# LeoQLi/DeepSIR

Hardware: AMD Instinct MI355X
Metric: registered pairs/sec (5k-pt 3DMatch-shaped synthetic pairs, 5 registration iterations, KNN pyramid included) (higher is better)
Workload: dtype f32 (GEMMs as fp16-pair MFMA, fp32 accumulate; index decisions exact fp32)

## Files before the change

deepsir_amd/csrc/kernels.h:

```cpp
#pragma once
#include <hip/hip_runtime.h>
#include <stdint.h>
#include <stdlib.h>

namespace dsir {

constexpr int kKnn = 16;

const char* tuning_env(const char* name);
inline bool tuning_flag(const char* name) { return tuning_env(name) != nullptr; }
inline long long tuning_int(const char* name, long long dflt) { const char* e = tuning_env(name); return e ? atoll(e) : dflt; }

#ifndef DSIR_GN_WORDS_DEFINED
#define DSIR_GN_WORDS_DEFINED
constexpr int kGnWords = 4;
#endif
struct GnRef {
  const double* stats;
  const float* gamma;
  const float* beta;
  int groups;
  double inv_count;
};

// ... 176 lines not shown
  Seg in = {};
  const float *W1 = nullptr;
  const float *W2 = nullptr, *b2 = nullptr;
  const float *W3 = nullptr, *b3 = nullptr;
  const float *W4 = nullptr, *b4 = nullptr;
  int ncls = 0, M = 0, clouds = 1;
  float* feat_out = nullptr;
  float* logits_out = nullptr;
  const void* Wh[4] = {nullptr, nullptr, nullptr, nullptr};
  const void* Wl[4] = {nullptr, nullptr, nullptr, nullptr};
};
bool launch_head_mlp(const HeadArgs& a, bool split, hipStream_t st);

struct AggArgs {
  const float* xyz = nullptr; int64_t xyz_cs = 0;
  const float* score = nullptr;
  const float* F = nullptr;
  const float *W1 = nullptr, *b1 = nullptr;
  const float *W2 = nullptr, *b2 = nullptr;
  const float *W3 = nullptr, *b3 = nullptr;
  const float *W4 = nullptr, *b4 = nullptr;
  const float *W5 = nullptr, *b5 = nullptr;
  const float *W6 = nullptr, *b6 = nullptr;
  float* desc = nullptr;
  int n = 0, clouds = 0;
  float* sq = nullptr;
  void* hi = nullptr;
  void* lo = nullptr;
  unsigned long long* packed_init = nullptr;
  const void* Wh[5] = {nullptr, nullptr, nullptr, nullptr, nullptr};
  const void* Wl[5] = {nullptr, nullptr, nullptr, nullptr, nullptr};
};
bool launch_agg_chain(const AggArgs& a, bool split, hipStream_t st);

struct FeatChainArgs {
  const float* X = nullptr;
  const float *W1 = nullptr, *b1 = nullptr;
  const float *W2 = nullptr, *b2 = nullptr;
  const float *W3 = nullptr, *b3 = nullptr;
  const void *W3h = nullptr, *W3l = nullptr;
  float* out0 = nullptr;
  float* out1 = nullptr;
  int split_cloud = 0;
  int n = 0, clouds = 0;
  int max_blocks = 0;
};
bool launch_feat_chain(const FeatChainArgs& a, hipStream_t st);
long long feat_chain_blocks(int clouds, int n);
void split_weights_f16(const float* w, size_t n, uint16_t* hi, uint16_t* lo);

size_t topk_scratch_bytes(int clouds, int n);
int launch_topk(const float* score, int clouds, int n, int k, int32_t* idx_out, float* score_out, void* scratch, hipStream_t st);
size_t scatter_plan_scratch_bytes(int64_t total);
int launch_scatter_plan(const int32_t* idx, int m, int clouds, int n, int32_t* order, int32_t* offsets, void* scratch, hipStream_t st);
void launch_gather_rows(const float* in, int64_t in_cloud_stride, int ld, const int32_t* idx, int C, int m, int clouds, float* out,
                        hipStream_t st);
void launch_gather_i32(const int32_t* in, int64_t in_cloud_stride, const int32_t* idx, int m, int clouds, int32_t* out,
                       hipStream_t st);
void launch_l2norm64(const float* x, int64_t rows, float* y, hipStream_t st);

void launch_residual_combine(const float* a, GnRef ga, const float* b, GnRef gb, int C, int rows, int clouds,
                             float* y, hipStream_t st);
void launch_gather_max(const float* in, int64_t in_cloud_stride, const int32_t* idx, int64_t idx_cloud_stride, int C,
                       int rows_out, int clouds, float* out, hipStream_t st);

void launch_gather_max_combine(const float* a, GnRef ga, const float* b, GnRef gb, int rows_in, const int32_t* idx,
                               int64_t idx_cloud_stride, int C, int rows_out, int clouds, float* out, hipStream_t st);

struct GmcArgs {
  const float* a; GnRef ga; const float* b; GnRef gb; int rows_in; const int32_t* idx; int64_t idx_cs; int C, rows_out; float* out; int bpc;
};
enum WalkKind { WK_TILE_SMALL = 0, WK_TILE_ATT2 = 1, WK_ATT_FULL64 = 2, WK_GMC = 3 };
struct WalkJob {
  int kind = 0;
  int v0 = 0, v1 = 0;
  int gx = 1, gy = 1;
  int dep = -1;
  GemmArgs gemm;
  AttPool16Args att;
  GmcArgs gmc = {};
};
constexpr int kWalkMaxPhases = 32;
constexpr int kWalkCtrWords = 2 * kWalkMaxPhases + 2;
struct WalkProgram {
  int nphases = 0, clouds = 0, wpc = 1;
  int flags = 0;
  unsigned* ctr = nullptr;
  unsigned long long* trace = nullptr;
  WalkJob job[kWalkMaxPhases];
};
bool walk_plan_gemm(const GemmArgs& a, WalkJob* out);
bool walk_plan_att_full(const AttPool16Args& a, int KH, int wpc, WalkJob* out);
bool walk_plan_gmc(const GmcArgs& a, int wpc, WalkJob* out);
void launch_walk(const WalkProgram& host, const WalkProgram* prog, hipStream_t st);

void launch_narrow_i64(const int64_t* src, int32_t* dst, int64_t n, hipStream_t st);

struct MemOp { void* dst; const void* src; size_t bytes; uint32_t fill; };
struct MemOps {
  static constexpr int kMax = 10;
  int n = 0;
  MemOp op[kMax];
  bool overflow = false;
  void fill(void* dst, size_t bytes, uint32_t word = 0) { if (dst && bytes) add(MemOp{dst, nullptr, bytes, word}); }
  void copy(void* dst, const void* src, size_t bytes) { if (dst && src && bytes) add(MemOp{dst, src, bytes, 0u}); }
  void add(const MemOp& o) { if (n < kMax) op[n++] = o; else overflow = true; }
};
void launch_mem_ops(const MemOps& m, hipStream_t st);

void launch_copy_idx_clamped(const int32_t* src, int64_t src_cloud_stride, int count, int limit, int clouds, int32_t* dst,
                             int64_t dst_cloud_stride, int32_t* flag, int flag_mod, hipStream_t st);
struct PyramidIdxCopy {
  const int32_t *neigh, *sub, *interp;
  int32_t *neigh_out, *sub_out, *interp_out;
  int S, S1, levels;
  int nl[6], off[6], soff[6];
  int32_t* flag; int flag_mod;
};
void launch_copy_pyramid_idx(const PyramidIdxCopy& a, int clouds, hipStream_t st);

void launch_knn16(const float* pts, int64_t cloud_stride, int stride, int n, int clouds, int32_t* out,
                  int64_t out_cloud_stride, hipStream_t st);
struct KnnSmallJobs {
  static constexpr int kMax = 8;
  struct Job {
    int kind;
    int n, n_support;
    int32_t* out;
    int64_t ocs;
    int b0;
  } job[kMax];
  int njobs;
};
bool knn16_takes_wave_kernel(int n, int clouds);
void launch_knn_small_levels(const float* pts, int64_t cloud_stride, int stride, int clouds, KnnSmallJobs& jobs, hipStream_t st);
size_t knn_grid_scratch_bytes(int clouds, int n);
void launch_knn16_grid(const float* pts, int64_t cloud_stride, int stride, int n, int clouds, int32_t* out,
                       int64_t out_cloud_stride, void* scratch, hipStream_t st);
bool knn16_grid_can_merge(int n);
void launch_knn16_grid_levels(const float* pts, int64_t cloud_stride, int stride, int nlev, const int* n, int clouds, int32_t* const* out,
                              int64_t out_cloud_stride, void* const* scratch, hipStream_t st);
void launch_nn1(const float* pts, int64_t cloud_stride, int stride, int n_query, int n_support, int clouds,
                int32_t* out, int64_t out_cloud_stride, hipStream_t st);
void launch_nn1_grid(int n_query, int n_support, int clouds, int32_t* out, int64_t out_cloud_stride, const void* grid_scratch,
                     const void* query_scratch, hipStream_t st);
void launch_copy_xyz(const float* pts, int64_t cloud_stride, int stride, int n, int clouds, float* out,
                     int64_t out_cloud_stride, hipStream_t st);
constexpr int kMaxLevels = 4;
struct PyramidLevels { int L; int nl[kMaxLevels + 1]; int off[kMaxLevels + 1]; int soff[kMaxLevels + 1]; int S, S1; };
void launch_copy_xyz_levels(const float* pts, int64_t cloud_stride, int stride, const PyramidLevels& lv, int clouds, float* xyz,
                            int64_t xyz_cs, hipStream_t st);
void launch_copy_sub_levels(const int32_t* neigh, int64_t neigh_cs, const PyramidLevels& lv, int clouds, int32_t* sub, int64_t sub_cs,
                            hipStream_t st);
void launch_copy_rows_i32(const int32_t* src, int64_t src_cloud_stride, int rows, int width, int clouds, int32_t* dst,
                          int64_t dst_cloud_stride, hipStream_t st);

struct ScoreScratch {
  float* red;
  float* prob;
  int32_t* label;
};
void launch_score(const float* feat, const float* logits, int ncls, const float* xyz, int64_t xyz_cloud_stride,
                  const int32_t* neigh, int64_t neigh_cloud_stride, int clouds, int n, ScoreScratch s, float* score,
                  int32_t* label_out, hipStream_t st, bool red_preset = false);

size_t nn_match_scratch_bytes(int pairs, int J, int K);
void launch_nn_match_ws(const float* a, const float* b, int pairs, int J, int K, int32_t* idx, void* scratch,
                        hipStream_t st, hipEvent_t ev0, hipEvent_t ev1, bool ref_norms_cached = false,
                        unsigned long long* tstamp = nullptr,
                        bool src_norms_ready = false);
void nn_match_scratch_layout(void* scratch, int pairs, int J, int K, float** sa, unsigned long long** packed);
void launch_nn_match_gated(const float* a, const float* b, const float* sa, const float* sb, int pairs, int J, int K,
                           unsigned long long* packed, const int32_t* gate, int gate_min, const int32_t* rowlist,
                           hipStream_t st);

void launch_sqnorm(const float* x, int64_t rows, float* out, hipStream_t st);

size_t nn_screen_scratch_bytes(int pairs, int J);
struct ScreenOrder {
  const int32_t* rows = nullptr;
  const int32_t* cols = nullptr;
  const void* bh = nullptr;
  const void* bl = nullptr;
  const float* sbp = nullptr;
  const int32_t* tlist = nullptr;
  const int32_t* tcount = nullptr;
  int tl_stride = 0;
  const int32_t* rborder = nullptr;
  int32_t* queue = nullptr;
  long long cand_rs = 0;
};
int nn_screen_rows_per_block(int J);
bool nn_prune_supported(int pairs, int J, int K);
size_t nn_prune_scratch_bytes(int pairs, int J, int K);
int launch_prune_ref(const float* ref_xyz, int64_t xyz_cloud_stride, const float* desc_ref, const void* bh, const void* bl, const float* sb,
                     int pairs, int J, int K, void* scratch, hipStream_t st);
int launch_prune_rows(const float* desc_src, const float* desc_ref, const void* ah, const void* al, const float* sa, const float* sb,
                      const int32_t* idx_prev, int pairs, int J, int K, void* scratch, hipStream_t st, ScreenOrder* ord, unsigned long long* acc);
void launch_split16(const float* x, int64_t rows, void* hi, void* lo, hipStream_t st, int32_t* bad = nullptr);
void launch_split16_norm(const float* x, int64_t rows, void* hi, void* lo, float* sq, hipStream_t st, int32_t* bad = nullptr);
void launch_nn_screen(const float* a, const float* b, const void* ah, const void* al, const void* bh, const void* bl,
                      const float* sa, const float* sb, int pairs, int J, int K, int32_t* idx, void* scratch, hipStream_t st,
                      hipEvent_t ev0 = nullptr, hipEvent_t ev1 = nullptr, unsigned long long* stats = nullptr,
                      bool keep_gate = false, const int32_t* bad = nullptr, unsigned long long* acc = nullptr,
                      hipEvent_t evk0 = nullptr, hipEvent_t evk1 = nullptr,
                      const ScreenOrder& ord = ScreenOrder());
int nn_screen_cap();
void launch_screen_bounds(const float* a, const float* b, const void* ah, const void* al, const void* bh, const void* bl,
                          const float* sa, const float* sb, int J, int K, float* lower, float* upper, float* exact, float* zacc,
                          hipStream_t st);
void launch_screen_export(const void* scratch, int J, float* thresh, int32_t* count, int32_t* code, float* lower, hipStream_t st);

struct KabschArgs {
  const float* src;
  const float* ref;
  const int32_t* idx;
  const float* w;
  int64_t src_stride, ref_stride;
  int sigmoid;
  int pairs, m;
  float* T;
  int32_t* invalid;
  float* src_out;
  int64_t src_out_stride;
  const float* T_prev;
  float* T_cum;
  int64_t T_stride;
  float* matched_out;
  int ref_ld;
  const int32_t* skip;
  double* part;
  int chunk_min;
  const int32_t* counts;
  const int32_t* ref_counts;
  int zero_freeze;
};
__host__ __device__ __forceinline__ int pair_rows(const int32_t* counts, int pair, int cap) {
  if (!counts) return cap;
  const int n = counts[pair];
  return n < 0 ? 0 : (n > cap ? cap : n);
}
constexpr int kKabschChunkedMin = 16384;
size_t kabsch_part_bytes(int pairs, int m, int chunk_min = 0);
void launch_kabsch(const KabschArgs& a, hipStream_t st);

enum class IcpSearch : int {
  Brute = 0,
  Grid = 1,
  GridUnordered = 2,
};
struct IcpArgs {
  const float* src; const float* ref;
  int pairs, J, K, stride;
  const int32_t* counts_src;
  const int32_t* counts_ref;
  float max_corr_dist; int max_iter; float rel_fitness, rel_rmse;
  const float* T_init; float* T_out;
  int estimator;
  const float* normals;
  int64_t normals_cs; int normals_ld;
  IcpSearch search;
  double* stats_out;
  double* stats5_out;
  int kernel; float kernel_scale;
};
size_t icp_scratch_bytes(const IcpArgs& a);
int launch_icp_refine(const IcpArgs& a, void* scratch, hipStream_t st);
size_t icp_corr_scratch_bytes(const IcpArgs& a);
int launch_icp_correspondences(const IcpArgs& a, int32_t* idx_out, float* d2_out, double* stats_out, void* scratch, hipStream_t st);

struct IcpGrid { const void* keys; const void* sorted; const int32_t* perm; const void* lat; };
size_t icp_grid_scratch_bytes(int pairs, int J, int K);
int icp_grid_build(const float* ref, int stride, const float* cur, int pairs, int J, int K, const int32_t* counts_src, const int32_t* counts_ref,
                   float r, bool order, void* scratch, hipStream_t st, IcpGrid* out);
void launch_icp_nn_grid(const IcpGrid& g, const float* cur, int pairs, int J, int K, const int32_t* counts_src, const int32_t* counts_ref, float r2,
                        int32_t* idx, float* d2, const int32_t* skip, hipStream_t st);
size_t cell_sort_tmp_bytes(int pairs, int n);
bool cell_sort_pairs(void* tmp, size_t tmp_bytes, const uint64_t* kin, uint64_t* kout, const uint32_t* vin, uint32_t* vout, int pairs, int n,
                     const int32_t* off, hipStream_t st);

void launch_corr_compact(const int32_t* ab, const int32_t* ba, int pairs, int J, int K, int mutual, int32_t* corr, int32_t* counts,
                         hipStream_t st);

void launch_pose_finetune(const float* src, const float* ref, const float* w, int sigmoid, int pairs, int m, const float* T_init,
                          float quant, int max_iter, float break_ratio, int max_break, float* T_out, double* stats,
                          hipStream_t st);

int launch_align_loss(const float* src, const float* ref, const int32_t* idx, const float* logits, const float* labels,
                      const float* T_gt, int P, int J, int K, int n_iter, int mse, float wt_pt, float wt_in, float discount,
                      float wt_pose, float* T_out, double* losses, float* grad, hipStream_t st, double* loss_part);

size_t voxel_downsample_scratch_bytes(int64_t total, int clouds);
int launch_voxel_downsample(const float* pts, const int64_t* offsets_host, int clouds, int stride, float voxel,
                            const float* crop_host, int cap, float* out, int32_t* counts, void* scratch, hipStream_t st,
                            const int32_t** bad_row_dev);
constexpr int32_t kVoxelNoBadRow = 0x7fffffff;
size_t resample_scratch_bytes(int clouds, int cap);
int launch_resample(const float* in, const int32_t* counts, int clouds, int cap, int stride, int k, int mode, uint64_t seed,
                    float* out, void* scratch, hipStream_t st);

void launch_eval_metrics(const float* pred, int64_t pred_stride, const float* gt, const float* src, const float* ref,
                         int pairs, int n, int stride, float rte_thresh, float rre_thresh, double* out, hipStream_t st);

size_t nn_topk_scratch_bytes(int pairs, int J, int K, int k);
int nn_topk_splits(int pairs, int J, int K, int k);
void launch_nn_topk(const float* a, const float* b, int pairs, int J, int K, int k, int32_t* idx, float* dist, void* scratch,
// ... 6 lines not shown
```

deepsir_amd/csrc/knn.hip:

```cpp
#include "kernels.h"
#include "device_utils.h"

namespace dsir {

namespace {

constexpr int QB = 64;
constexpr int NW = 4;
constexpr int TILE = 256;
constexpr int QCAP = 16;

__device__ __forceinline__ float sqdist(float qx, float qy, float qz, const float4& s) {
  const float dx = __fsub_rn(s.x, qx), dy = __fsub_rn(s.y, qy), dz = __fsub_rn(s.z, qz);
  return __fadd_rn(__fadd_rn(__fmul_rn(dx, dx), __fmul_rn(dy, dy)), __fmul_rn(dz, dz));
}

struct Top16 {
  float d[kKnn];
  int i[kKnn];
  __device__ __forceinline__ void init() {
#pragma unroll
    for (int t = 0; t < kKnn; ++t) { d[t] = INFINITY; i[t] = -1; }
  }
  __device__ __forceinline__ void insert(float dist, int idx) {
// ... 74 lines not shown
    for (int j0 = 0; j0 < cnt; j0 += 8) {
      float dd[8];
#pragma unroll
      for (int u = 0; u < 8; ++u) {
        const float4 s = tile[w][j0 + u];
        dd[u] = (j0 + u < cnt) ? sqdist(qx, qy, qz, s) : INFINITY;
      }
#pragma unroll
      for (int u = 0; u < 8; ++u)
        if (dd[u] < thr) { qd[w][nq][lane] = dd[u]; qi[w][nq][lane] = s_begin + t0 + j0 + u; ++nq; }
      if (__any(nq > QCAP - 8)) flush();
    }
    __syncthreads();
  }
  flush();
  if (w > 0) {
#pragma unroll
    for (int t = 0; t < kKnn; ++t) { md[w - 1][t][lane] = top.d[t]; mi[w - 1][t][lane] = top.i[t]; }
  }
  __syncthreads();
  if (w == 0 && q < n) {
#pragma unroll
    for (int s = 0; s < NW - 1; ++s) {
      float ld[kKnn];
      int li[kKnn];
#pragma unroll
      for (int t = 0; t < kKnn; ++t) { ld[t] = md[s][t][lane]; li[t] = mi[s][t][lane]; }
      top.merge_sorted(ld, li);
    }
    int32_t* o = out + (int64_t)q * kKnn;
#pragma unroll
    for (int t = 0; t < kKnn; ++t) top.i[t] = top.i[t] < 0 ? q : top.i[t];
#pragma unroll
    for (int t = 0; t < kKnn; t += 4) *reinterpret_cast<int4*>(o + t) = make_int4(top.i[t], top.i[t + 1], top.i[t + 2], top.i[t + 3]);
  }
}
__global__ __launch_bounds__(QB * NW) void knn16_kernel(const float* __restrict__ pts, int64_t cs, int stride, int n,
                                                        int32_t* __restrict__ out, int64_t ocs) {
  __shared__ Knn16Smem sm;
  knn16_body(pts + blockIdx.y * cs, stride, n, out + blockIdx.y * ocs, blockIdx.x, sm);
}

constexpr int WQ_MAX = 16;
__device__ __forceinline__ void knn16_wave_body(const float* __restrict__ P, int stride, int n, int32_t* __restrict__ out, int bx) {
  const int lane = threadIdx.x & 63;
  const int q = bx * 4 + (threadIdx.x >> 6);
  if (q >= n) return;
  const float qx = P[(int64_t)q * stride], qy = P[(int64_t)q * stride + 1], qz = P[(int64_t)q * stride + 2];
  unsigned long long key[WQ_MAX];
#pragma unroll
  for (int i = 0; i < WQ_MAX; ++i) {
    const int j = lane + 64 * i;
    key[i] = ~0ull;
    if (j < n) {
      float4 s;
      s.x = P[(int64_t)j * stride]; s.y = P[(int64_t)j * stride + 1]; s.z = P[(int64_t)j * stride + 2]; s.w = 0.f;
      const float d = sqdist(qx, qy, qz, s);
      if (d == d && d < INFINITY) key[i] = ((unsigned long long)__float_as_uint(d) << 32) | (unsigned)j;
    }
  }
  int mine = -1;
  for (int t = 0; t < kKnn; ++t) {
    unsigned long long m = key[0];
#pragma unroll
    for (int i = 1; i < WQ_MAX; ++i) m = key[i] < m ? key[i] : m;
    unsigned long long w = m;
#pragma unroll
    for (int o = 32; o > 0; o >>= 1) {
      const unsigned long long v = __shfl_xor(w, o);
      w = v < w ? v : w;
    }
    if (lane == t) mine = w == ~0ull ? q : (int)(unsigned)(w & 0xffffffffull);
#pragma unroll
    for (int i = 0; i < WQ_MAX; ++i) key[i] = key[i] == w ? ~0ull : key[i];
  }
  if (lane < kKnn) out[(int64_t)q * kKnn + lane] = mine;
}
__global__ __launch_bounds__(256) void knn16_wave_kernel(const float* __restrict__ pts, int64_t cs, int stride, int n,
                                                         int32_t* __restrict__ out, int64_t ocs) {
  knn16_wave_body(pts + blockIdx.y * cs, stride, n, out + blockIdx.y * ocs, blockIdx.x);
}

struct Nn1Smem {
  float4 tile[NW][TILE];
  float md[NW][QB];
  int mi[NW][QB];
};
__device__ __forceinline__ void nn1_body(const float* __restrict__ P, int stride, int n_query, int n_support, int32_t* __restrict__ out, int bx,
                                         Nn1Smem& sm) {
  auto& tile = sm.tile;
  auto& md = sm.md;
  auto& mi = sm.mi;
  const int lane = threadIdx.x & 63, w = threadIdx.x >> 6;
  const int q = bx * QB + lane;
  float qx = 0.f, qy = 0.f, qz = 0.f;
  if (q < n_query) { qx = P[(int64_t)q * stride]; qy = P[(int64_t)q * stride + 1]; qz = P[(int64_t)q * stride + 2]; }
  const int slice = (n_support + NW - 1) / NW;
  const int s_begin = w * slice;
  const int s_end = min(n_support, s_begin + slice);
  float bd = INFINITY;
  int bi = -1;
  for (int t0 = 0; t0 < slice; t0 += TILE) {
#pragma unroll
    for (int r = 0; r < TILE / 64; ++r) {
      const int j = s_begin + t0 + r * 64 + lane;
      float4 v = make_float4(0.f, 0.f, 0.f, 0.f);
      if (j < s_end) { v.x = P[(int64_t)j * stride]; v.y = P[(int64_t)j * stride + 1]; v.z = P[(int64_t)j * stride + 2]; }
      tile[w][r * 64 + lane] = v;
    }
    __syncthreads();
    const int cnt = max(0, min(TILE, s_end - (s_begin + t0)));
    for (int j = 0; j < cnt; ++j) {
      const float d = sqdist(qx, qy, qz, tile[w][j]);
      if (d < bd) { bd = d; bi = s_begin + t0 + j; }
    }
    __syncthreads();
  }
  md[w][lane] = bd; mi[w][lane] = bi;
  __syncthreads();
  if (w == 0 && q < n_query) {
#pragma unroll
    for (int s = 1; s < NW; ++s) {
      const float d = md[s][lane];
      if (d < bd) { bd = d; bi = mi[s][lane]; }
    }
    out[q] = bi < 0 ? 0 : bi;
  }
}
__global__ __launch_bounds__(QB * NW) void nn1_kernel(const float* __restrict__ pts, int64_t cs, int stride, int n_query,
                                                      int n_support, int32_t* __restrict__ out, int64_t ocs) {
  __shared__ Nn1Smem sm;
  nn1_body(pts + blockIdx.y * cs, stride, n_query, n_support, out + blockIdx.y * ocs, blockIdx.x, sm);
}

template <bool K16>
struct SmallSmem { union { Nn1Smem nn1; Knn16Smem k16; }; };
template <>
struct SmallSmem<false> { Nn1Smem nn1; };
template <bool K16>
__global__ __launch_bounds__(256) void knn_small_levels_kernel(const float* __restrict__ pts, int64_t cs, int stride, const KnnSmallJobs J) {
  static_assert(QB * NW == 256, "the bodies run 256 threads");
  __shared__ SmallSmem<K16> sm;
  int j = 0;
#pragma unroll
  for (int k = 1; k < KnnSmallJobs::kMax; ++k) j += (k < J.njobs && (int)blockIdx.x >= J.job[k].b0) ? 1 : 0;
  const KnnSmallJobs::Job& jb = J.job[j];
  const int bx = (int)blockIdx.x - jb.b0;
  const float* P = pts + blockIdx.y * cs;
  if (jb.kind == 0) nn1_body(P, stride, jb.n, jb.n_support, jb.out + blockIdx.y * jb.ocs, bx, sm.nn1);
  else if (jb.kind == 1) knn16_wave_body(P, stride, jb.n, jb.out + blockIdx.y * jb.ocs, bx);
  else if constexpr (K16) knn16_body(P, stride, jb.n, jb.out + blockIdx.y * jb.ocs, bx, sm.k16);
}

}

void launch_knn16(const float* pts, int64_t cs, int stride, int n, int clouds, int32_t* out, int64_t ocs, hipStream_t st) {
  if (knn16_takes_wave_kernel(n, clouds)) {
    hipLaunchKernelGGL(knn16_wave_kernel, dim3((n + 3) / 4, clouds), dim3(256), 0, st, pts, cs, stride, n, out, ocs);
    return;
  }
  dim3 grid((n + QB - 1) / QB, clouds);
  hipLaunchKernelGGL(knn16_kernel, grid, dim3(QB * NW), 0, st, pts, cs, stride, n, out, ocs);
}

bool knn16_takes_wave_kernel(int n, int clouds) { return n <= 64 * WQ_MAX && (int64_t)clouds * n <= 4096; }

void launch_knn_small_levels(const float* pts, int64_t cs, int stride, int clouds, KnnSmallJobs& J, hipStream_t st) {
  KnnSmallJobs S{};
  for (int kind = 2; kind >= 0; --kind)
    for (int k = 0; k < J.njobs; ++k)
      if (J.job[k].kind == kind) S.job[S.njobs++] = J.job[k];
  int b = 0;
  bool k16 = false;
  for (int k = 0; k < S.njobs; ++k) {
    S.job[k].b0 = b;
    b += S.job[k].kind == 1 ? (S.job[k].n + 3) / 4 : (S.job[k].n + QB - 1) / QB;
    k16 = k16 || S.job[k].kind == 2;
  }
  J = S;
  if (b == 0 || clouds <= 0) return;
  if (k16) hipLaunchKernelGGL(knn_small_levels_kernel<true>, dim3(b, clouds), dim3(256), 0, st, pts, cs, stride, S);
  else hipLaunchKernelGGL(knn_small_levels_kernel<false>, dim3(b, clouds), dim3(256), 0, st, pts, cs, stride, S);
}

void launch_nn1(const float* pts, int64_t cs, int stride, int n_query, int n_support, int clouds, int32_t* out,
                int64_t ocs, hipStream_t st) {
  dim3 grid((n_query + QB - 1) / QB, clouds);
  hipLaunchKernelGGL(nn1_kernel, grid, dim3(QB * NW), 0, st, pts, cs, stride, n_query, n_support, out, ocs);
}

}
```

deepsir_amd/csrc/schedule.hip:

```cpp
#include <cstddef>
#include <cstring>
#include <vector>

#include "engine_ctx.h"

namespace dsir {

namespace {
void level_sizes(const dsir_cfg& cfg, int n, int* nl) {
  nl[0] = n;
  for (int l = 0; l < cfg.num_layers; ++l) nl[l + 1] = nl[l] / cfg.sub_sampling_ratio[l];
}
}

void fill_pyramid_layout(const dsir_cfg& cfg, int clouds, int n, Pyramid& p) {
  p.clouds = clouds; p.n = n;
  level_sizes(cfg, n, p.nl);
  p.off[0] = 0; p.soff[0] = 0;
  for (int l = 0; l < cfg.num_layers; ++l) { p.off[l + 1] = p.off[l] + p.nl[l]; p.soff[l + 1] = p.soff[l] + p.nl[l + 1]; }
  p.S = p.off[cfg.num_layers]; p.S1 = p.soff[cfg.num_layers];
}

int gn_max_contributions(const dsir_cfg& g, int n, int flags) {
  const bool ppf = (flags & DSIR_FLAG_PPF) != 0;
// ... 530 lines not shown
    x = samp;
  }
  x = s.mlp2d(w.mid, Sched::seg_of(skips.back()), nullptr, py.nl[L], true);
  for (int j = 0; j < L; ++j) {
    const int lvl = L - 1 - j;
    const Act& sk = skips[skips.size() - 2 - j];
    const Seg s0 = Sched::seg_of(sk);
    const Seg s1 = Sched::seg_of(x, py.interp + py.off[lvl], interp_cs);
    if (s.rec && lvl < walk_from) { s.rec_flush(); s.rec = nullptr; }
    x = s.mlp2d(w.dec[j], s0, &s1, py.nl[lvl], true);
  }
  if (s.rec) { s.rec_flush(); s.rec = nullptr; }
  if (s.rec_error) return 1;
  const int n0 = py.nl[0];
  bool fused = false;
  static const bool no_head = tuning_flag("DSIR_NO_HEAD");
  if (logits_out && !no_head &&w.dec_out == 32 && g.out_feat_dim == 64 && w.fc[0].cout == 64 && w.fc[1].cout == 32) {
    HeadArgs h;
    h.in = Sched::seg_of(x);
    h.W1 = w.out_w; h.W2 = w.fc[0].W; h.b2 = w.fc[0].b; h.W3 = w.fc[1].W; h.b3 = w.fc[1].b; h.W4 = w.fc[2].W; h.b4 = w.fc[2].b;
    h.ncls = w.ncls; h.M = n0; h.clouds = py.clouds; h.feat_out = feat_out; h.logits_out = logits_out;
    if (c->ws.overflow) return overflow_fail(c, "workspace exhausted in randla_forward (raise max_points / max_pairs)");
    if (c->agg_split) {
      for (int k = 0; k < 4; ++k) { h.Wh[k] = w.head_wh[k]; h.Wl[k] = w.head_wl[k]; }
      fused = launch_head_mlp(h, true, st);
    }
    if (!fused) fused = launch_head_mlp(h, false, st);
  }
  LinW ow; ow.W = w.out_w; ow.b = nullptr; ow.cin = w.dec_out; ow.cout = g.out_feat_dim;
  Act feat;
  if (!fused) feat = s.linear(ow, Sched::seg_of(x), nullptr, n0, EPI_LINEAR, feat_out);
  if (logits_out && !fused) {
    Act h = s.linear(w.fc[0], Sched::seg_of(feat), nullptr, n0, EPI_ACT);
    h = s.linear(w.fc[1], Sched::seg_of(h), nullptr, n0, EPI_ACT);
    s.linear(w.fc[2], Sched::seg_of(h), nullptr, n0, EPI_LINEAR, logits_out);
  }
  if (c->ws.overflow) return overflow_fail(c, "workspace exhausted in randla_forward (raise max_points / max_pairs)");
  if (cache) cache->valid = true;
  return 0;
}

namespace {
bool feat_chain_wanted(int clouds, int n) {
  static const bool off = tuning_flag("DSIR_NO_FEAT_CHAIN");
  static const long long min_blocks = tuning_int("DSIR_FEAT_CHAIN_MIN_BLOCKS", 64);
  return !off && feat_chain_blocks(clouds, n) >= min_blocks;
}
bool mlp_feat_chain(dsir_ctx* c, const float* feat0, int clouds, int n, float* out0, float* out1, int split_cloud, int max_blocks) {
  const LinW* m = c->net.mlp_feat;
  if (m[0].cin != 64 || m[0].cout != 64 || m[1].cin != 64 || m[1].cout != 128 || m[2].cin != 128 || m[2].cout != 64) return false;
  FeatChainArgs a;
  a.X = feat0;
  a.W1 = m[0].W; a.b1 = m[0].b; a.W2 = m[1].W; a.b2 = m[1].b; a.W3 = m[2].W; a.b3 = m[2].b;
  GemmArgs last;
  last.W = m[2].W;
  Sched{c, c->stream, clouds}.split_of(last);
  a.W3h = last.Wh; a.W3l = last.Wl;
  a.out0 = out0; a.out1 = out1; a.split_cloud = split_cloud; a.n = n; a.clouds = clouds; a.max_blocks = max_blocks;
  return launch_feat_chain(a, c->stream);
}
bool takes_fused(FeatForm form, int clouds, int n) { return form == FeatForm::Fused || (form == FeatForm::Auto && feat_chain_wanted(clouds, n)); }
}

float* run_mlp_feat(dsir_ctx* c, const float* feat0, int clouds, int n, float* out, FeatForm form, int max_blocks) {
  Sched s{c, c->stream, clouds};
  const NetW& w = c->net;
  if (takes_fused(form, clouds, n)) {
    float* y = out ? out : c->ws.get<float>((size_t)clouds * n * 64);
    if (c->ws.overflow) return y;
    if (mlp_feat_chain(c, feat0, clouds, n, y, nullptr, clouds, max_blocks)) return y;
    if (form == FeatForm::Fused) return nullptr;
    out = y;
  }
  Act h = s.linear(w.mlp_feat[0], plain_seg(feat0, (int64_t)n * 64, 64, 64), nullptr, n, EPI_ACT);
  h = s.linear(w.mlp_feat[1], Sched::seg_of(h), nullptr, n, EPI_ACT);
  h = s.linear(w.mlp_feat[2], Sched::seg_of(h), nullptr, n, EPI_LINEAR, out);
  return h.p;
}
float* run_mlp_feat_pair(dsir_ctx* c, const float* feat0, int P, int n, float* out_a, FeatForm form, int max_blocks) {
  float* out_b = c->ws.get<float>((size_t)P * n * 64);
  if (c->ws.overflow) return out_b;
  if (takes_fused(form, 2 * P, n) && mlp_feat_chain(c, feat0, 2 * P, n, out_a, out_b, P, max_blocks)) return out_b;
  if (form == FeatForm::Fused) return nullptr;
  run_mlp_feat(c, feat0, P, n, out_a, FeatForm::Three);
  run_mlp_feat(c, feat0 + (size_t)P * n * 64, P, n, out_b, FeatForm::Three);
  return out_b;
}
int run_mlp_feat_probe(dsir_ctx* c, const float* feat0, int clouds, int n, int fused, int max_blocks, float* out) {
  if (fused == 2) {
    const int P = clouds / 2;
    const float* half = run_mlp_feat_pair(c, feat0, P, n, out, FeatForm::Fused, max_blocks);
    if (c->ws.overflow) return overflow_fail(c, "workspace exhausted in mlp_feat_probe");
    if (!half) return fail(c, "mlp_feat_probe: the fused launch does not take this configuration");
    HIP_OK(c, hipMemcpyAsync(out + (size_t)P * n * 64, half, sizeof(float) * P * n * 64, hipMemcpyDeviceToDevice, c->stream));
    return 0;
  }
  const float* y = run_mlp_feat(c, feat0, clouds, n, out, fused ? FeatForm::Fused : FeatForm::Three, max_blocks);
  if (c->ws.overflow) {
    if (c->call.sched_error) return fail(c, "mlp_feat_probe: %s", c->call.sched_error);
    return overflow_fail(c, "workspace exhausted in mlp_feat_probe");
  }
  if (!y) return fail(c, "mlp_feat_probe: the fused launch does not take this configuration");
  return 0;
}
bool run_att_proj(dsir_ctx* c, const float* xyz, int64_t xyz_cs, const float* score, const float* F, int clouds, int n,
                  float* desc, const AggExtras* ex) {
  Sched s{c, c->stream, clouds};
  const NetW& w = c->net;
  static const bool no_agg = tuning_flag("DSIR_NO_AGG");
  const LinW* m = w.mlp_att;
  if (!no_agg && m[0].cin == 4 && m[0].cout == 32 && m[1].cout == 64 && m[2].cout == 128 && m[3].cout == 256 &&
      m[4].cout == 64 && w.mlp_proj.cin == 64 && w.mlp_proj.cout == 64) {
    AggArgs a;
    a.xyz = xyz; a.xyz_cs = xyz_cs; a.score = score; a.F = F;
    a.W1 = m[0].W; a.b1 = m[0].b; a.W2 = m[1].W; a.b2 = m[1].b; a.W3 = m[2].W; a.b3 = m[2].b;
    a.W4 = m[3].W; a.b4 = m[3].b; a.W5 = m[4].W; a.b5 = m[4].b; a.W6 = w.mlp_proj.W; a.b6 = w.mlp_proj.b;
    a.desc = desc; a.n = n; a.clouds = clouds;
    static const bool no_fuse = tuning_flag("DSIR_NO_AGG_EXTRAS");
    if (c->agg_split) {
      for (int k = 0; k < 5; ++k) { a.Wh[k] = c->agg_wh[k]; a.Wl[k] = c->agg_wl[k]; }
      if (ex && !no_fuse) { a.sq = ex->sq; a.hi = ex->hi; a.lo = ex->lo; a.packed_init = ex->packed_init; }
      if (launch_agg_chain(a, true, c->stream)) return ex && !no_fuse;
      a.sq = nullptr; a.hi = a.lo = nullptr; a.packed_init = nullptr;
    }
    if (launch_agg_chain(a, false, c->stream)) return false;
  }
  const Seg sx = plain_seg(xyz, xyz_cs, 3, 3);
  const Seg ss = plain_seg(score, n, 1, 1);
  Act h = s.linear(w.mlp_att[0], sx, &ss, n, EPI_ACT);
  for (int k = 1; k < 4; ++k) h = s.linear(w.mlp_att[k], Sched::seg_of(h), nullptr, n, EPI_ACT);
  h = s.linear(w.mlp_att[4], Sched::seg_of(h), nullptr, n, EPI_LINEAR, nullptr, F);
  s.linear(w.mlp_proj, Sched::seg_of(h), nullptr, n, EPI_L2NORM, desc);
  return false;
}

int build_pyramid(dsir_ctx* c, const float* points, int stride, int clouds, int n, float* xyz, int32_t* neigh,
                  int32_t* sub, int32_t* interp) {
  const dsir_cfg& g = c->cfg;
  Pyramid p;
  fill_pyramid_layout(g, clouds, n, p);
  if (p.nl[g.num_layers - 1] < kKnn)
    return fail(c, "cloud too small: level %d has %d < %d points (need n >= %d)", g.num_layers - 1,
                p.nl[g.num_layers - 1], kKnn, kKnn * 64);
  hipStream_t st = c->stream;
  const int64_t xyz_cs = (int64_t)p.S * 3, neigh_cs = (int64_t)p.S * kKnn, sub_cs = (int64_t)p.S1 * kKnn;
  PyramidLevels lv{};
  lv.L = g.num_layers; lv.S = p.S; lv.S1 = p.S1;
  for (int l = 0; l <= g.num_layers; ++l) { lv.nl[l] = p.nl[l]; lv.off[l] = p.off[l]; lv.soff[l] = p.soff[l]; }
  launch_copy_xyz_levels(points, (int64_t)n * stride, stride, lv, clouds, xyz, xyz_cs, st);
  static const bool no_grid = tuning_flag("DSIR_NO_GRID");
  static const int grid_min = (int)tuning_int("DSIR_GRID_MIN", 1024);
  static const bool no_nn1_grid = tuning_flag("DSIR_NO_NN1_GRID");
  static const long long nn1_grid_min = tuning_int("DSIR_NN1_GRID_MIN", 65536);
  auto nn1_by_grid = [&](int l) {
    return !no_grid && !no_nn1_grid && l + 1 < g.num_layers && p.nl[l + 1] >= grid_min && (int64_t)clouds * p.nl[l] >= nn1_grid_min;
  };
  const size_t mark = c->ws.mark();
  const void* prev_scratch = nullptr;
  static const bool no_merge = tuning_flag("DSIR_NO_PYRAMID_MERGE");
  if (!no_merge && g.num_layers <= KnnSmallJobs::kMax / 2) {
    int ngrid = 0, gn[4], grid_of[8];
    int32_t* gout[4];
    KnnSmallJobs jobs{};
    bool ok = true;
    for (int l = 0; l < g.num_layers && ok; ++l) {
      grid_of[l] = -1;
      if (p.nl[l] >= grid_min && !no_grid) {
        ok = knn16_grid_can_merge(p.nl[l]) && ngrid < 4;
        if (ok) { gn[ngrid] = p.nl[l]; gout[ngrid] = neigh + (int64_t)p.off[l] * kKnn; grid_of[l] = ngrid++; }
      } else {
        jobs.job[jobs.njobs++] = {knn16_takes_wave_kernel(p.nl[l], clouds) ? 1 : 2, p.nl[l], 0, neigh + (int64_t)p.off[l] * kKnn, neigh_cs, 0};
      }
      if (!nn1_by_grid(l)) jobs.job[jobs.njobs++] = {0, p.nl[l], p.nl[l + 1], interp + p.off[l], (int64_t)p.S, 0};
    }
    if (ok) {
      void* gscr[4];
      for (int k = 0; k < ngrid; ++k) gscr[k] = c->ws.raw(knn_grid_scratch_bytes(clouds, gn[k]));
      if (c->ws.overflow) return fail(c, "workspace exhausted in the KNN pyramid");
      if (ngrid) launch_knn16_grid_levels(points, (int64_t)n * stride, stride, ngrid, gn, clouds, gout, neigh_cs, gscr, st);
      launch_knn_small_levels(points, (int64_t)n * stride, stride, clouds, jobs, st);
      for (int l = 0; l + 1 < g.num_layers; ++l)
        if (nn1_by_grid(l))
          launch_nn1_grid(p.nl[l], p.nl[l + 1], clouds, interp + p.off[l], p.S, gscr[grid_of[l + 1]], gscr[grid_of[l]], st);
      c->ws.release(mark);
      launch_copy_sub_levels(neigh, neigh_cs, lv, clouds, sub, sub_cs, st);
      return 0;
    }
  }
  for (int l = 0; l < g.num_layers; ++l) {
    if (p.nl[l] >= grid_min && !no_grid) {
      void* scratch = c->ws.raw(knn_grid_scratch_bytes(clouds, p.nl[l]));
      if (c->ws.overflow) return fail(c, "workspace exhausted in the KNN pyramid");
      launch_knn16_grid(points, (int64_t)n * stride, stride, p.nl[l], clouds, neigh + (int64_t)p.off[l] * kKnn, neigh_cs,
                        scratch, st);
      if (l > 0 && nn1_by_grid(l - 1))
        launch_nn1_grid(p.nl[l - 1], p.nl[l], clouds, interp + p.off[l - 1], p.S, scratch, prev_scratch, st);
      prev_scratch = scratch;
    } else {
      prev_scratch = nullptr;
      launch_knn16(points, (int64_t)n * stride, stride, p.nl[l], clouds, neigh + (int64_t)p.off[l] * kKnn, neigh_cs, st);
    }
    if (!nn1_by_grid(l)) launch_nn1(points, (int64_t)n * stride, stride, p.nl[l], p.nl[l + 1], clouds, interp + p.off[l], p.S, st);
  }
  c->ws.release(mark);
  launch_copy_sub_levels(neigh, neigh_cs, lv, clouds, sub, sub_cs, st);
  return 0;
}

}
```

Measured before the change: 5262.

## Derive upsampling nearest neighbours from existing KNN lists instead of searching

Adds a kernel that copies the subsampled neighbour rows and, in the same pass, takes each point's upsampling (interp) index as the first of its 16 nearest neighbours whose index falls inside the next coarser level. Because the coarse level is a prefix of the fine one, that neighbour is the exact nearest coarse point whenever one is among the 16. Only points with no such neighbour, or padded rows, fall back to a brute-force wave-wide scan. This removes the separate nn1 and nn1_grid searches from the pyramid build. The cost is a divergent fallback loop for uncovered points, and ties between equal distances may resolve differently than before.

After: 5315, median of 6. 1.0% higher.

```diff
diff --git a/deepsir_amd/csrc/kernels.h b/deepsir_amd/csrc/kernels.h
--- a/deepsir_amd/csrc/kernels.h
+++ b/deepsir_amd/csrc/kernels.h
@@ -352,6 +352,8 @@
                             int64_t xyz_cs, hipStream_t st);
 void launch_copy_sub_levels(const int32_t* neigh, int64_t neigh_cs, const PyramidLevels& lv, int clouds, int32_t* sub, int64_t sub_cs,
                             hipStream_t st);
+void launch_interp_lists(const float* pts, int64_t cloud_stride, int stride, const int32_t* neigh, int64_t neigh_cs, const PyramidLevels& lv,
+                         int clouds, int32_t* sub, int64_t sub_cs, int32_t* interp, int64_t interp_cs, hipStream_t st);
 void launch_copy_rows_i32(const int32_t* src, int64_t src_cloud_stride, int rows, int width, int clouds, int32_t* dst,
                           int64_t dst_cloud_stride, hipStream_t st);
 
diff --git a/deepsir_amd/csrc/knn.hip b/deepsir_amd/csrc/knn.hip
--- a/deepsir_amd/csrc/knn.hip
+++ b/deepsir_amd/csrc/knn.hip
@@ -250,6 +250,65 @@
   else if constexpr (K16) knn16_body(P, stride, jb.n, jb.out + blockIdx.y * jb.ocs, bx, sm.k16);
 }
 
+__global__ __launch_bounds__(256) void interp_lists_kernel(const float* __restrict__ pts, int64_t cs, int stride,
+                                                           const int32_t* __restrict__ neigh, int64_t ncs, const PyramidLevels lv,
+                                                           int32_t* __restrict__ sub, int64_t scs, int32_t* __restrict__ interp, int64_t ics) {
+  const int cloud = blockIdx.y;
+  const int lane = threadIdx.x & 63, part = threadIdx.x & 3;
+  const int p = (int)((blockIdx.x * 256 + threadIdx.x) >> 2);
+  const bool valid = p < lv.S;
+  int l = 0;
+#pragma unroll
+  for (int k = 1; k < kMaxLevels; ++k) l += (k < lv.L && p >= lv.off[k]) ? 1 : 0;
+  const int q = p - lv.off[l];
+  const int m = lv.nl[l + 1];
+  int4 e = make_int4(-1, -1, -1, -1);
+  if (valid) e = *reinterpret_cast<const int4*>(neigh + cloud * ncs + (int64_t)p * kKnn + part * 4);
+  if (valid && q < m) *reinterpret_cast<int4*>(sub + cloud * scs + (int64_t)(lv.soff[l] + q) * kKnn + part * 4) = e;
+  int c = -1;
+  c = (unsigned)e.w < (unsigned)m ? e.w : c;
+  c = (unsigned)e.z < (unsigned)m ? e.z : c;
+  c = (unsigned)e.y < (unsigned)m ? e.y : c;
+  c = (unsigned)e.x < (unsigned)m ? e.x : c;
+  const unsigned long long has = __ballot(c >= 0);
+  const unsigned long long padded = __ballot(part == 0 && e.x == q && e.y == q);
+  const int base = lane & ~3;
+  const unsigned mine = (unsigned)(has >> base) & 15u;
+  int ans = __shfl(c, base + (mine ? __ffs((int)mine) - 1 : 0));
+  if (!mine || ((padded >> base) & 1)) ans = -1;
+  unsigned long long need = __ballot(valid && part == 0 && ans < 0);
+  const float* P = pts + cloud * cs;
+  while (need) {
+    const int src = __ffsll((long long)need) - 1;
+    need &= need - 1;
+    const int fq = __shfl(q, src), fm = __shfl(m, src);
+    const float qx = P[(int64_t)fq * stride], qy = P[(int64_t)fq * stride + 1], qz = P[(int64_t)fq * stride + 2];
+    float bd = INFINITY;
+    int bi = -1;
+    for (int j0 = lane; j0 < fm + lane; j0 += 256) {
+      float4 s[4];
+#pragma unroll
+      for (int u = 0; u < 4; ++u) {
+        const int64_t j = min(j0 + 64 * u, fm - 1);
+        s[u] = make_float4(P[j * stride], P[j * stride + 1], P[j * stride + 2], 0.f);
+      }
+#pragma unroll
+      for (int u = 0; u < 4; ++u) {
+        const float d = sqdist(qx, qy, qz, s[u]);
+        if (j0 + 64 * u < fm && d < bd) { bd = d; bi = j0 + 64 * u; }
+      }
+    }
+#pragma unroll
+    for (int o = 32; o > 0; o >>= 1) {
+      const float od = __shfl_xor(bd, o);
+      const int oi = __shfl_xor(bi, o);
+      if (od < bd || (od == bd && oi < bi)) { bd = od; bi = oi; }
+    }
+    if (lane == src) ans = bi < 0 ? 0 : bi;
+  }
+  if (valid && part == 0) interp[cloud * ics + p] = ans;
+}
+
 }
 
 void launch_knn16(const float* pts, int64_t cs, int stride, int n, int clouds, int32_t* out, int64_t ocs, hipStream_t st) {
@@ -281,6 +340,13 @@
   else hipLaunchKernelGGL(knn_small_levels_kernel<false>, dim3(b, clouds), dim3(256), 0, st, pts, cs, stride, S);
 }
 
+void launch_interp_lists(const float* pts, int64_t cs, int stride, const int32_t* neigh, int64_t ncs, const PyramidLevels& lv, int clouds,
+                         int32_t* sub, int64_t scs, int32_t* interp, int64_t ics, hipStream_t st) {
+  if (lv.S <= 0 || clouds <= 0) return;
+  hipLaunchKernelGGL(interp_lists_kernel, dim3((lv.S + 63) / 64, clouds), dim3(256), 0, st, pts, cs, stride, neigh, ncs, lv, sub, scs,
+                     interp, ics);
+}
+
 void launch_nn1(const float* pts, int64_t cs, int stride, int n_query, int n_support, int clouds, int32_t* out,
                 int64_t ocs, hipStream_t st) {
   dim3 grid((n_query + QB - 1) / QB, clouds);
diff --git a/deepsir_amd/csrc/schedule.hip b/deepsir_amd/csrc/schedule.hip
--- a/deepsir_amd/csrc/schedule.hip
+++ b/deepsir_amd/csrc/schedule.hip
@@ -706,6 +706,11 @@
   static const int grid_min = (int)tuning_int("DSIR_GRID_MIN", 1024);
   static const bool no_nn1_grid = tuning_flag("DSIR_NO_NN1_GRID");
   static const long long nn1_grid_min = tuning_int("DSIR_NN1_GRID_MIN", 65536);
+  static const bool nn1_search = tuning_flag("DSIR_NO_INTERP_LISTS");
+  auto finish = [&]() {
+    if (nn1_search) launch_copy_sub_levels(neigh, neigh_cs, lv, clouds, sub, sub_cs, st);
+    else launch_interp_lists(points, (int64_t)n * stride, stride, neigh, neigh_cs, lv, clouds, sub, sub_cs, interp, p.S, st);
+  };
   auto nn1_by_grid = [&](int l) {
     return !no_grid && !no_nn1_grid && l + 1 < g.num_layers && p.nl[l + 1] >= grid_min && (int64_t)clouds * p.nl[l] >= nn1_grid_min;
   };
@@ -725,7 +730,7 @@
       } else {
         jobs.job[jobs.njobs++] = {knn16_takes_wave_kernel(p.nl[l], clouds) ? 1 : 2, p.nl[l], 0, neigh + (int64_t)p.off[l] * kKnn, neigh_cs, 0};
       }
-      if (!nn1_by_grid(l)) jobs.job[jobs.njobs++] = {0, p.nl[l], p.nl[l + 1], interp + p.off[l], (int64_t)p.S, 0};
+      if (nn1_search && !nn1_by_grid(l)) jobs.job[jobs.njobs++] = {0, p.nl[l], p.nl[l + 1], interp + p.off[l], (int64_t)p.S, 0};
     }
     if (ok) {
       void* gscr[4];
@@ -734,10 +739,10 @@
       if (ngrid) launch_knn16_grid_levels(points, (int64_t)n * stride, stride, ngrid, gn, clouds, gout, neigh_cs, gscr, st);
       launch_knn_small_levels(points, (int64_t)n * stride, stride, clouds, jobs, st);
       for (int l = 0; l + 1 < g.num_layers; ++l)
-        if (nn1_by_grid(l))
+        if (nn1_search && nn1_by_grid(l))
           launch_nn1_grid(p.nl[l], p.nl[l + 1], clouds, interp + p.off[l], p.S, gscr[grid_of[l + 1]], gscr[grid_of[l]], st);
       c->ws.release(mark);
-      launch_copy_sub_levels(neigh, neigh_cs, lv, clouds, sub, sub_cs, st);
+      finish();
       return 0;
     }
   }
@@ -747,17 +752,17 @@
       if (c->ws.overflow) return fail(c, "workspace exhausted in the KNN pyramid");
       launch_knn16_grid(points, (int64_t)n * stride, stride, p.nl[l], clouds, neigh + (int64_t)p.off[l] * kKnn, neigh_cs,
                         scratch, st);
-      if (l > 0 && nn1_by_grid(l - 1))
+      if (nn1_search && l > 0 && nn1_by_grid(l - 1))
         launch_nn1_grid(p.nl[l - 1], p.nl[l], clouds, interp + p.off[l - 1], p.S, scratch, prev_scratch, st);
       prev_scratch = scratch;
     } else {
       prev_scratch = nullptr;
       launch_knn16(points, (int64_t)n * stride, stride, p.nl[l], clouds, neigh + (int64_t)p.off[l] * kKnn, neigh_cs, st);
     }
-    if (!nn1_by_grid(l)) launch_nn1(points, (int64_t)n * stride, stride, p.nl[l], p.nl[l + 1], clouds, interp + p.off[l], p.S, st);
+    if (nn1_search && !nn1_by_grid(l)) launch_nn1(points, (int64_t)n * stride, stride, p.nl[l], p.nl[l + 1], clouds, interp + p.off[l], p.S, st);
   }
   c->ws.release(mark);
-  launch_copy_sub_levels(neigh, neigh_cs, lv, clouds, sub, sub_cs, st);
+  finish();
   return 0;
 }
 
```
